# taithenguyen/ppls

Measured on AMD Instinct MI355X. Metric: accepted subintervals/sec + FP64 F-evals/sec at 1/2/4/8 MI355X, EPSILON=1e-10, higher is better.
Workload: dtype f64

## Files before the change

ppls_amd/csrc/aq_shape.h:

```cpp
#pragma once

#if defined(__HIPCC__)
#define AQ_SHAPE_HD __host__ __device__
#else
#define AQ_SHAPE_HD
#endif

namespace aq {

#ifndef AQ_PT
#define AQ_PT 768
#endif
#ifndef AQ_WCAP
#define AQ_WCAP 256
#endif
constexpr int PT = AQ_PT;
constexpr int NW = PT / 64;
constexpr int WCAP = AQ_WCAP;
#ifndef AQ_LONE_NW
#define AQ_LONE_NW 8
#endif
#ifndef AQ_S_W
#define AQ_S_W 2
#endif
constexpr int S_W = AQ_S_W;
#ifndef AQ_S_W1
#define AQ_S_W1 2
#endif
AQ_SHAPE_HD constexpr int seed_depth(unsigned long long V) {
    return V <= 1ull ? AQ_S_W1 : 63 - __builtin_clzll(V) + S_W;
}
AQ_SHAPE_HD constexpr unsigned seed_nb(int D, unsigned long long V) {
    if (V <= 1ull) return 1u << D;
    unsigned nb = 1u << (D - (63 - __builtin_clzll(V)));
    while (nb > 1u && (unsigned long long)(nb - 1u) * V >= (1ull << D)) --nb;
    return nb;
}
AQ_SHAPE_HD constexpr int seed_depth_job(unsigned long long V) {
    return (unsigned long long)(seed_depth(V) + 2) * seed_nb(seed_depth(V) + 1, V) <= 64ull
        ? seed_depth(V) + 1 : seed_depth(V);
}
constexpr int PCU_MAXK = 12;
constexpr int STATIC_MAXK = 16;
constexpr int MAXK = 1 << 18;
constexpr int NSLOTS = MAXK;
constexpr int SYNC_SLOT = NSLOTS;
constexpr int NPARTS = 16384;
#ifndef AQ_GSPLIT_DEFAULT
#define AQ_GSPLIT_DEFAULT 192
#endif
constexpr int DEFAULT_GSPLIT = AQ_GSPLIT_DEFAULT;
// ... 14 lines not shown
```

ppls_amd/csrc/aq_stream.h:

```cpp
#pragma once
#include "aq_device.h"
#include "aq_shape.h"
#include "aq_xsum.h"

namespace aq {

typedef double f64x2 __attribute__((ext_vector_type(2)));

constexpr int PCAP = 128;
constexpr int DT_STRIDE = 2;
constexpr int LREC = NW * WCAP + PCAP;
constexpr int POOL0 = NW * WCAP;
constexpr int CH = PCAP;
struct DtField {
    unsigned* p;
    __device__ __forceinline__ unsigned& operator[](unsigned j) const { return p[DT_STRIDE * j]; }
    __device__ __forceinline__ DtField operator+(unsigned o) const { return DtField{p + DT_STRIDE * o}; }
};
#ifndef AQ_JOB_RUN_MAX
#define AQ_JOB_RUN_MAX 16
#endif
constexpr int JOB_RUN_MAX = AQ_JOB_RUN_MAX;
#ifndef AQ_GSS_DIV
#define AQ_GSS_DIV 2
#endif
constexpr unsigned GSS_DIV = AQ_GSS_DIV;
#ifndef AQ_HEAP_SEED
#define AQ_HEAP_SEED 1
#endif
constexpr bool HEAP_SEED = AQ_HEAP_SEED != 0;
constexpr int HEAP_D = 4;
constexpr unsigned HEAP_NODES = (2u << HEAP_D) - 1u;
static_assert(HEAP_NODES + 2u <= 64u, "the heap seeding path is one node per lane");
__device__ __forceinline__ unsigned div_small(unsigned q, unsigned nb, float rnb) {
    unsigned d = (unsigned)((float)q * rnb);
    d += (d + 1u) * nb <= q ? 1u : 0u;
    d -= d * nb > q ? 1u : 0u;
    return d;
}
#ifndef AQ_GIVE_MIN
#define AQ_GIVE_MIN 96
#endif
constexpr int GIVE_MIN = AQ_GIVE_MIN;
constexpr int DONATE_MIN = 64;
#ifndef AQ_POLL_ROUNDS
// ... 189 lines not shown
    unsigned long long* cu_acc;
    Chunk* chunks;
    Cellar* cellar;
    unsigned* ready;
    LaunchHint* hint;
    int per_cu;
    int static_jobs;
    double2 kbounds[PCU_MAXK];
    int adaptive;
    const double* theta;
};
static_assert(sizeof(StreamParams) == 384, "the kernels' hidden arguments follow the block: a larger one moves them in every instance");

enum : int {
    DG_T_START = 0, DG_T_SEEDED, DG_T_FIRST_LEAD, DG_T_EXIT, DG_ROUNDS, DG_TASKS, DG_CHUNKS_OUT, DG_CHUNKS_IN,
    DG_RECORDS_OUT, DG_T_WAIT, DG_LEADS, DG_SEEDS, DG_POOL_PUSH, DG_CU, DG_RECORDS_IN, DG_ACTIVE_LANES,
    DG_C_ROUND, DG_C_EVAL, DG_POOL_TAKE, DG_LOCK_SPINS, DG_T_LAST_ROUND, DG_SPILL_RECORDS, DG_MAX_RING, DG_C_SEED,
    DG_SEED_CALLS, DG_FLUSHES, DG_MAX_CELLAR, DG_C_IDLE, DG_C_LOCK, DG_C_SHARE, DG_GIVE, DG_CELLAR_IN,
    DG_CELLAR_OUT, DG_C_REFILL, DG_C_LOOP, DG_ACTIVE_TASKS, DG_PREFETCH, DG_T_INIT, DG_T_DONE, DG_T_FOLD,
    DG_T_BROKE, DG_T_FLUSHED, DG_C_P1_CLASS, DG_C_P1_WALK, DG_C_P1_F, DG_T_SEED_IN, DG_T_CLASS, DG_POLLS,
    DIAG_WORDS = 48
};

struct WgState {
    int lock;
    unsigned pbot, ptop;
    int idle;
    int phase;
    int busy_token;
    unsigned exited;
    unsigned long long tasks;
};

struct LdsPairs {
    double* a;
    double* b;
    double* fa;
    double* fm;
    double* fb;
    DtField dt;
};

__device__ __forceinline__ void wave_lock(int* lock, unsigned lane, unsigned long long& spins) {
    if (lane == 0) {
        int expect = 0;
        while (!__hip_atomic_compare_exchange_strong(lock, &expect, 1, __ATOMIC_ACQUIRE, __ATOMIC_RELAXED,
                                                     __HIP_MEMORY_SCOPE_WORKGROUP)) {
            expect = 0;
            ++spins;
            __builtin_amdgcn_s_sleep(1);
        }
    }
    __builtin_amdgcn_wave_barrier();
    __builtin_amdgcn_fence(__ATOMIC_ACQUIRE, "workgroup");
}

__device__ __forceinline__ void wave_unlock(int* lock, unsigned lane) {
    __builtin_amdgcn_fence(__ATOMIC_RELEASE, "workgroup");
    __builtin_amdgcn_wave_barrier();
    if (lane == 0) __hip_atomic_store(lock, 0, __ATOMIC_RELEASE, __HIP_MEMORY_SCOPE_WORKGROUP);
    __builtin_amdgcn_wave_barrier();
}

__device__ __forceinline__ void copy_pair(const LdsPairs& R, unsigned i, unsigned j) {
    const double a = R.a[i], b = R.b[i], fa = R.fa[i], fm = R.fm[i], fb = R.fb[i];
    const unsigned dt = R.dt[i];
    R.a[j] = a; R.b[j] = b; R.fa[j] = fa; R.fm[j] = fm; R.fb[j] = fb; R.dt[j] = dt;
}

template <typename SrcIdx>
__device__ __forceinline__ void publish_chunk(const StreamParams& P, const LdsPairs& R, unsigned slot, unsigned k,
                                              SrcIdx src, unsigned lane) {
    Chunk* __restrict__ c = P.chunks + slot;
    for (unsigned i = lane; i < k; i += 64) {
        const unsigned j = src(i);
        st_wt(&c->a[i], R.a[j]); st_wt(&c->b[i], R.b[j]);
        st_wt(&c->fa[i], R.fa[j]); st_wt(&c->fm[i], R.fm[j]); st_wt(&c->fb[i], R.fb[j]);
        st_wt(&c->dt[i], R.dt[j]);
    }
    if (lane == 0) st_wt(&c->count, k);
    asm volatile("s_waitcnt vmcnt(0)" ::: "memory");
    if (lane == 0) st_wt(&P.ready[(size_t)slot * READY_STRIDE], P.epoch);
}

struct Acc {
    double hi, lo;
    unsigned tasks, leaves, maxd;
    unsigned ut, ul;
    unsigned maxdt;
    double r = 0.0;
};

template <bool ERR>
struct ErrAcc {};
template <>
struct ErrAcc<true> {
    double sg = 0.0, ab = 0.0;
};

template <int FID, bool PCU, bool ERR = false>
__device__ __forceinline__ void flush_acc(const StreamParams& P, Acc& a, int tag, unsigned lane, WgState& S,
                                          unsigned long long* pc, double2* wdd, int wdd_stride, long long* xsa,
                                          long long* xsb, ErrAcc<ERR>& ea, double2* werr) {
    dd_add(a.hi, a.lo, a.r);
    a.r = 0.0;
    if (uni(a.ut) != 0u || __ballot(a.tasks != 0u) != 0ull) {
        double hi = area_scale<FID>() * a.hi, lo = area_scale<FID>() * a.lo;
#if AQ_FLUSHX == 1
        const unsigned t = a.ut + 1u, l = a.ul, m = 1u;
#elif AQ_FLUSHX == 3
        const unsigned mdt = wave_max_full(a.maxdt);
// ... 86 lines not shown
    const unsigned long long a64 = (unsigned long long)(base + p);
    const unsigned long long addr = ((unsigned long long)(unsigned)__builtin_amdgcn_readfirstlane((int)(a64 >> 32)) << 32) |
                                    (unsigned)__builtin_amdgcn_readfirstlane((int)(unsigned)a64);
    u32x4 r;
    asm volatile("s_load_dwordx4 %0, %1, 0x0\n\ts_waitcnt lgkmcnt(0)" : "=s"(r) : "s"(addr) : "memory");
    return make_double2(__hiloint2double((int)r.y, (int)r.x), __hiloint2double((int)r.w, (int)r.z));
}

typedef unsigned u32x2 __attribute__((ext_vector_type(2)));
template <int FID>
__device__ __forceinline__ void sload_theta(Theta<FID>& th, const double* base, int p) {
    if constexpr (FID == F_PARAM) {
        constexpr int NP = param::nparams;
        const unsigned long long a64 = (unsigned long long)(base + (size_t)p * NP);
        const unsigned long long addr = ((unsigned long long)(unsigned)__builtin_amdgcn_readfirstlane((int)(a64 >> 32)) << 32) |
                                        (unsigned)__builtin_amdgcn_readfirstlane((int)(unsigned)a64);
#pragma unroll
        for (int i = 0; i < NP; i += 2) {
            const unsigned long long ai = addr + 8ull * (unsigned)i;
            if (i + 1 < NP) {
                u32x4 r;
                asm volatile("s_load_dwordx4 %0, %1, 0x0\n\ts_waitcnt lgkmcnt(0)" : "=s"(r) : "s"(ai) : "memory");
                th.v[i] = __hiloint2double((int)r.y, (int)r.x);
                th.v[i + 1 < NP ? i + 1 : i] = __hiloint2double((int)r.w, (int)r.z);
            } else {
                u32x2 r;
                asm volatile("s_load_dwordx2 %0, %1, 0x0\n\ts_waitcnt lgkmcnt(0)" : "=s"(r) : "s"(ai) : "memory");
                th.v[i] = __hiloint2double((int)r.y, (int)r.x);
            }
        }
    }
}

static_assert(LREC * 8 == 50 * 512, "the pair moves assume 50 x 512 B per field");
__device__ __forceinline__ void lds_pop6_masked(unsigned long long m, unsigned addr, unsigned addr2, double& a,
                                                double& b, double& fa, double& fm, double& fb, double& dw) {
    unsigned long long saved;
    asm volatile(
        "s_mov_b64 %6, exec\n\t"
        "s_mov_b64 exec, %7\n\t"
        "ds_read_b64 %0, %8\n\t"
        "ds_read_b64 %1, %8 offset:25600\n\t"
        "ds_read_b64 %2, %8 offset:51200\n\t"
        "ds_read_b64 %3, %9\n\t"
        "ds_read_b64 %4, %9 offset:25600\n\t"
        "ds_read_b64 %5, %9 offset:51200\n\t"
        "s_mov_b64 exec, %6\n\t"
        "s_waitcnt lgkmcnt(0)"
        : "+v"(a), "+v"(b), "+v"(fa), "+v"(fm), "+v"(fb), "+v"(dw), "=&s"(saved)
        : "s"(m), "v"(addr), "v"(addr2)
        : "memory");
}
__device__ __forceinline__ void lds_push6_masked(unsigned long long m, unsigned addr, double x0, double x1, double x2,
                                                 double x3, double x4, double x5) {
    unsigned long long saved;
    asm volatile(
        "s_mov_b64 %0, exec\n\t"
        "s_mov_b64 exec, %1\n\t"
        "ds_write2st64_b64 %2, %3, %4 offset1:50\n\t"
        "ds_write2st64_b64 %2, %5, %6 offset0:100 offset1:150\n\t"
        "ds_write2st64_b64 %2, %7, %8 offset0:200 offset1:250\n\t"
        "s_mov_b64 exec, %0"
        : "=&s"(saved)
        : "s"(m), "v"(addr), "v"(x0), "v"(x1), "v"(x2), "v"(x3), "v"(x4), "v"(x5)
        : "memory");
}
struct PairRegs {
    f64x2 ab, ff, fd;
};
__device__ __forceinline__ void lds_issue6(unsigned addr, PairRegs& r) {
    asm volatile(
        "ds_read2st64_b64 %0, %3 offset1:50\n\t"
        "ds_read2st64_b64 %1, %3 offset0:100 offset1:150\n\t"
        "ds_read2st64_b64 %2, %3 offset0:200 offset1:250"
        : "=&v"(r.ab), "=&v"(r.ff), "=&v"(r.fd)
        : "v"(addr)
        : "memory");
}
__device__ __forceinline__ void lds_wait6(PairRegs& r) {
    asm volatile("s_waitcnt lgkmcnt(0)" : "+v"(r.ab), "+v"(r.ff), "+v"(r.fd) : : "memory");
}
__device__ __forceinline__ void lds_store6(unsigned addr, const PairRegs& r) {
    asm volatile(
        "ds_write2st64_b64 %0, %1, %2 offset1:50\n\t"
        "ds_write2st64_b64 %0, %3, %4 offset0:100 offset1:150\n\t"
        "ds_write2st64_b64 %0, %5, %6 offset0:200 offset1:250"
        :
        : "v"(addr), "v"(r.ab.x), "v"(r.ab.y), "v"(r.ff.x), "v"(r.ff.y), "v"(r.fd.x), "v"(r.fd.y)
        : "memory");
}
__device__ __forceinline__ PairRegs chunk_load(const CellarChunk* ch, unsigned lane) {
    return PairRegs{ch->ab[lane], ch->ff[lane], ch->fd[lane]};
}
__device__ __forceinline__ void chunk_store(CellarChunk* ch, unsigned lane, const PairRegs& r) {
    ch->ab[lane] = r.ab;
    ch->ff[lane] = r.ff;
    ch->fd[lane] = r.fd;
}
__device__ __forceinline__ unsigned ring_addr(unsigned ring8, unsigned i, unsigned vmask) {
    return ((i << 3) & vmask) | ring8;
}
__device__ __forceinline__ unsigned ring_slot(unsigned i) { return i % (unsigned)WCAP; }
__device__ __forceinline__ unsigned ring_wrap(unsigned v) {
    if constexpr ((WCAP & (WCAP - 1)) == 0) return v & (unsigned)(WCAP - 1);
    else return min(v, v - (unsigned)WCAP);
}

#if AQ_STAMPS
__device__ unsigned long long g_aq_stamps[MAXG * NW * ST_STRIDE];
#endif

template <int FID, bool HIST, bool DIAG, bool PCU, int NWT = NW, bool HEAPS = false, bool ERR = false>
__global__ __launch_bounds__(NWT * 64) void k_stream(StreamParams P) {
    static_assert(!ERR || (!HIST && !DIAG), "ERR launches keep no histograms and no diagnostics");
    constexpr int PTT = NWT * 64;
    static_assert(NWT >= 4 && NWT <= NW && NWT % 4 == 0, "whole waves per SIMD, within the LDS rings");
    static_assert(NWT <= 16, "the exit's area sum runs over one DPP row of lanes (PCU_AREA)");
    constexpr bool WIDE = AQ_WIDE_TAB && FID == F_COSH4 && !PCU;
    constexpr int TAB_FRONT = WIDE ? 256 * 16 / 8 : 0;
    __shared__ double s_lds[TAB_FRONT + 6 * LREC];
    double* const s_pr = s_lds + TAB_FRONT;
    __shared__ ExpEntry tab_own[WIDE ? 1 : ftab_entries<FID>()];
    ExpEntry* const tab = WIDE ? reinterpret_cast<ExpEntry*>(s_lds) : tab_own;
    const DtField s_dt{reinterpret_cast<unsigned*>(s_pr + 5 * LREC)};
    double* const s_a = s_pr;
    double* const s_b = s_pr + LREC;
    double* const s_fa = s_pr + 2 * LREC;
    double* const s_fm = s_pr + 3 * LREC;
    double* const s_fb = s_pr + 4 * LREC;
    __shared__ WgState S;
    __shared__ unsigned long long s_pc[PCU ? 3 * PCU_ROW : 1];
    __shared__ double2 s_wdd[PCU ? PCU_ROW * NWT : 1];
    __shared__ double2 s_werr[PCU && ERR ? PCU_ROW * NWT : 1];
    __shared__ unsigned long long s_dg[DIAG ? DIAG_WORDS : 1];

    const unsigned tid = threadIdx.x;
    const unsigned lane = lane_id();
    const unsigned wid = __builtin_amdgcn_readfirstlane(tid >> 6);
    const unsigned bid = __builtin_amdgcn_readfirstlane(blockIdx.x);
    QCtl* __restrict__ qc = P.q;
    const LdsPairs R{s_a, s_b, s_fa, s_fm, s_fb, s_dt};
    const unsigned pr_base = (unsigned)(uintptr_t)s_pr;
    const unsigned long long t_entry = (DIAG || AQ_STAMPS) ? rtc() : 0ull;
    unsigned long long stp[ST_N] = {};
    auto stamp = [&](int k) {
        if constexpr (AQ_STAMPS && !DIAG) { if (!stp[k]) stp[k] = rtc(); }
    };
    stp[ST_ENTRY] = t_entry;
    if constexpr (AQ_STAMPS && !DIAG) {
        asm volatile("" :: "s"(P.eps), "s"(P.shares), "s"(P.nprob), "s"(P.kbounds[0].x));
        stamp(ST_KARG);
    }
    ExpPair tv{};
    if (FID != F_SIN_RECIP && tid < (WIDE ? 256u : 128u)) tv = reinterpret_cast<const ExpPair*>(kExpTabBits)[tid & 127u];
    static_assert(FID != F_SIN_RECIP || AQ_SINCOS_TAB_N <= PTT, "one sin-table entry per thread");
    double sv = 0.0;
    if (FID == F_SIN_RECIP && tid < (unsigned)AQ_SINCOS_TAB_N) sv = kSinCosTab[tid];
    stamp(ST_PRE);
    if (bid == 0)
        for (unsigned i = tid; i < (unsigned)(sizeof(QCtl) / 4); i += PTT) reinterpret_cast<unsigned*>(P.q_next)[i] = 0u;
    if (tid == 0) {
        S.lock = 0; S.pbot = 0; S.ptop = 0; S.idle = 0; S.phase = 0; S.busy_token = 1;
        S.exited = 0; S.tasks = 0;
    }
    if (PCU && tid < 3u * PCU_ROW) s_pc[tid] = 0ull;
    if (PCU)
        for (unsigned i = tid; i < (unsigned)(PCU_ROW * NWT); i += PTT) s_wdd[i] = make_double2(0.0, 0.0);
    if constexpr (PCU && ERR)
        for (unsigned i = tid; i < (unsigned)(PCU_ROW * NWT); i += PTT) s_werr[i] = make_double2(0.0, 0.0);
    if (DIAG) {
        for (unsigned i = tid; i < DIAG_WORDS; i += PTT) s_dg[i] = (i == DG_T_FIRST_LEAD) ? ~0ull : 0ull;
    }
    if (FID == F_SIN_RECIP) {
        if (tid < (unsigned)AQ_SINCOS_TAB_N) reinterpret_cast<double*>(tab)[tid] = sv;
// ... 7 lines not shown

    const double eps = P.eps;
    const double eps2 = eps / area_scale<FID>();
    const int max_depth = P.max_depth;
    unsigned shares_main = (unsigned)P.shares;
    int D_main = P.D;
    unsigned long long per_hint = 0;
    if (!PCU && (P.adaptive & 1)) {
        unsigned h = uni(__hip_atomic_load(&P.hint->shares_next, __ATOMIC_RELAXED, __HIP_MEMORY_SCOPE_AGENT));
        if (h) {
            if constexpr (HEAPS) {
                const unsigned long long per =
                    (P.adaptive & 4) ? __hip_atomic_load(&P.hint->per_next, __ATOMIC_RELAXED, __HIP_MEMORY_SCOPE_AGENT)
                                     : (h >= 2u ? (unsigned long long)h * TASKS_PER_JOB : 0ull);
                const unsigned fill = (gridDim.x * (unsigned)NWT + (unsigned)P.nprob - 1u) / (unsigned)P.nprob;
                const unsigned long long cap = per / MIN_JOB_TASKS;
                h = uni(max(h, (unsigned)min((unsigned long long)fill, cap)));
                per_hint = per;
            }
            shares_main = h;
            D_main = seed_depth_job((unsigned long long)h * (unsigned long long)P.nshards);
        }
    }
    const unsigned W = gridDim.x * (unsigned)NWT;
    const unsigned w_all = bid * (unsigned)NWT + wid;
    const unsigned grp = bid % (unsigned)NGROUP;
    const unsigned grp_size = (gridDim.x - grp + (unsigned)NGROUP - 1u) / (unsigned)NGROUP;
    const int t0 = (int)min(gridDim.x, (unsigned)NGROUP);
    const unsigned tail_from = (!PCU && shares_main >= 8u) ? (unsigned)P.tail_from : (unsigned)P.nprob;
    const unsigned shares_tail = min(shares_main * (unsigned)P.tail_mult, W);
    const int D_tail = seed_depth_job((unsigned long long)shares_tail * (unsigned long long)P.nshards);
    const unsigned main_jobs = tail_from * shares_main;
    const unsigned total_jobs = main_jobs + ((unsigned)P.nprob - tail_from) * shares_tail;
    const unsigned base = wid * WCAP;
    long long* const xs_a = reinterpret_cast<long long*>(s_a + base + (WCAP - 64));
    long long* const xs_b = reinterpret_cast<long long*>(s_b + base + (WCAP - 64));
    const unsigned ring8 = pr_base + base * 8u;
    __builtin_assume((ring8 & (unsigned)(WCAP * 8 - 1)) == 0u);
    unsigned ring_vmask = (unsigned)((WCAP - 1) << 3);
    asm volatile("" : "+v"(ring_vmask));

    Acc acc{0.0, 0.0, 0u, 0u, 0u, 0u, 0u, 0u};
    ErrAcc<ERR> eacc;
    auto err_leaf = [&](double d) {
        if constexpr (ERR) {
            eacc.sg += d / area_scale<FID>();
            eacc.ab += fabs(d) / area_scale<FID>();
        }
    };
    int tag = 0;
    Theta<FID> th{};
    sload_theta<FID>(th, P.theta, tag);
    unsigned ctop = 0;
    Cellar* __restrict__ cel = P.cellar + w_all;
    const bool static_jobs = PCU || P.static_jobs != 0;
    unsigned job = (static_jobs || HEAPS) ? wid * gridDim.x + bid : w_all;
    bool job_pending = false;
    unsigned claim = 0;
    unsigned jpc = (!static_jobs && shares_main == 1u && P.nshards == 1 && JOB_RUN_MAX > 1)
                       ? max(1u, min((unsigned)JOB_RUN_MAX, total_jobs / (4u * W)))
                       : 1u;
    if constexpr (HEAPS) {
        if (per_hint) jpc = uni(max(1u, min(jpc, (unsigned)min((unsigned long long)TASKS_PER_JOB / per_hint, 64ull))));
    }
    unsigned job_end = job + 1u;
    unsigned claim_n = jpc;
    unsigned err = 0;
    bool mixed = false;
    unsigned top = 0, bot = 0;
    bool counted_idle = false;
// ... 83 lines not shown
                }
            }
            if (job_pending) {
                job = W + uni(__shfl(claim, 0, 64));
                job_end = job + claim_n;
                job_pending = false;

            }
            unsigned k = 0;
            int ptag = 0;
            bool lead = false, seed = false;
            int phase = 0;
            bool counted_now = false;
            const bool pool_empty = uni(__hip_atomic_load(&S.ptop, __ATOMIC_RELAXED, __HIP_MEMORY_SCOPE_WORKGROUP)) ==
                                    uni(__hip_atomic_load(&S.pbot, __ATOMIC_RELAXED, __HIP_MEMORY_SCOPE_WORKGROUP));
            if (job < total_jobs && (fresh || pool_empty)) {
                seed = true;
            } else if (!counted_idle && !job_pending && job >= total_jobs && pool_empty) {
                stamp(ST_IDLE);
                unsigned old = 0;
                if (lane == 0) old = __hip_atomic_fetch_add(&S.idle, 1, __ATOMIC_RELAXED, __HIP_MEMORY_SCOPE_WORKGROUP);
                old = uni(__shfl(old, 0, 64));
                counted_idle = true;
                counted_now = old + 1u != (unsigned)NWT;
            }
            if (!seed && !counted_now) {
                wave_lock(&S.lock, lane, lock_spins);
                {
                    const unsigned avail = uni(S.ptop - S.pbot);
                    phase = uni(S.phase);
                    if (avail > 0) {
                        k = min(avail, (unsigned)REFILL);
                        const unsigned pb = S.pbot;
                        ptag = (int)uni(dt_tag(s_dt[POOL0 + (pb & (PCAP - 1))]));
                        for (unsigned q0 = 0; q0 < k; q0 += 64) {
                            const unsigned q = q0 + lane;
                            const unsigned long long bad =
                                __ballot(q < k && (int)dt_tag(s_dt[POOL0 + ((pb + q) & (PCAP - 1))]) != ptag);
                            if (bad) {
                                k = q0 + (unsigned)__builtin_ctzll(bad);
                                break;
                            }
                        }
                        for (unsigned i = lane; i < k; i += 64) copy_pair(R, POOL0 + ((pb + i) & (PCAP - 1)), base + i);
                        if (lane == 0) {
                            S.pbot = pb + k;
                            if (counted_idle) __hip_atomic_fetch_add(&S.idle, -1, __ATOMIC_RELAXED, __HIP_MEMORY_SCOPE_WORKGROUP);
                        }
                        __builtin_amdgcn_wave_barrier();
                        counted_idle = false;
                    } else if (job < total_jobs) {
                        seed = true;
                    } else {
                        if (!counted_idle) {
                            stamp(ST_IDLE);
                            if (lane == 0) __hip_atomic_fetch_add(&S.idle, 1, __ATOMIC_RELAXED, __HIP_MEMORY_SCOPE_WORKGROUP);
                            __builtin_amdgcn_wave_barrier();
                            counted_idle = true;
                        }
                        __builtin_amdgcn_wave_barrier();
                        if (phase == 0 && uni(__hip_atomic_load(&S.idle, __ATOMIC_RELAXED, __HIP_MEMORY_SCOPE_WORKGROUP)) == NWT) {
                            lead = true;
                            if (lane == 0) S.phase = 1;
                            __builtin_amdgcn_wave_barrier();
                        }
                    }
                }
                wave_unlock(&S.lock, lane);
            }
            fresh = false;
            if constexpr (DIAG) {
                if (lane == 0) {
                    if (k) atomicAdd(&s_dg[DG_POOL_TAKE], (unsigned long long)k);
                    atomicAdd(&s_dg[DG_C_IDLE], clk() - ci);
                }
            }
            if (k) {
// ... 43 lines not shown
                    for (unsigned d = 0; d < nlev; ++d) col0 |= 1ull << (d * nb);
                    colmask = uni(col0) << (lane - div_small(lane, nb, nb_rcp) * nb);
                }
                unsigned long long cf0 = 0;
                if constexpr (AQ_STAMPS && !DIAG) cf0 = clk();
                if (p != tag) {
                    flush_acc<FID, PCU, ERR>(P, acc, tag, lane, S, s_pc, s_wdd + wid, NWT, xs_a, xs_b, eacc, s_werr + wid);
                    tag = p;
                    sload_theta<FID>(th, P.theta, tag);
                }
                if constexpr (AQ_STAMPS && !DIAG) {
                    const unsigned long long cf1 = clk();
                    stp[ST_CF] += cf1 - cf0;
                    cf0 = cf1;
                }
                const double2 ab = PCU ? P.kbounds[p] : sload_bounds(P.bounds, p);
                if constexpr (AQ_STAMPS && !DIAG) stp[ST_CBD] += clk() - cf0;
                if (static_jobs) {
                    job += W;
                } else if (total_jobs > W) {
                    if (job + 1u < job_end) {
                        ++job;
                    } else {
                        const unsigned left = total_jobs > job + 1u ? total_jobs - job - 1u : 0u;
                        claim_n = jpc > 1u && GSS_DIV ? max(1u, min(jpc, left / (GSS_DIV * W))) : jpc;
                        if (lane == 0) claim = g_add(&qc->jobs.v, claim_n);
                        job_pending = true;
                    }
                } else {
                    job = total_jobs;
                }
                const double A = ab.x, B = ab.y;
                if constexpr (AQ_STAMPS && !DIAG) { asm volatile("" :: "s"(A)); stamp(ST_CLASS); }
                double* fm = s_a + base;
                double* leafa = s_b + base;
                const DtField flag = s_dt + base;
                [[maybe_unused]] double* dleafa = s_fa + base;
                auto position = [&](unsigned kk, bool& valid) -> unsigned long long {
                    const unsigned long long o = (kk & 1u) ? (unsigned long long)(V - 1 - vw) : (unsigned long long)vw;
                    const unsigned long long j = (unsigned long long)kk * V + o;
                    valid = j < npos_total;
                    return j;
                };
                unsigned long long cp1 = 0, cp2 = 0;
                bool alive = false, alive2 = false;
                double l = A, r = B, fl = 0.0, fr = 0.0, mid = 0.0, fmid = 0.0;
                double l2 = A, r2 = B, fl2 = 0.0, fr2 = 0.0, fmid2 = 0.0;
                int Ds = D;
                if (HEAP_SEED && HEAPS && V == 1u) {
                    Ds = HEAP_D;
                    const unsigned q = lane;
                    const bool isnode = q < HEAP_NODES;
                    const unsigned d = isnode ? 31u - (unsigned)__builtin_clz(q + 1u) : 0u;
                    const unsigned k = isnode ? q + 1u - (1u << d) : 0u;
                    unsigned li = HEAP_NODES, ri = HEAP_NODES + 1u;
                    for (unsigned i = 0; i < d; ++i) {
                        const double mm = (l + r) / 2;
                        const unsigned anc = (1u << i) - 1u + (k >> (d - i));
                        if ((k >> (d - 1u - i)) & 1u) { l = mm; li = anc; } else { r = mm; ri = anc; }
                    }
                    mid = (l + r) / 2;
                    if (q < HEAP_NODES + 2u) {
                        fmid = integrand<FID>(isnode ? mid : (q == HEAP_NODES ? A : B), tab, th);
                        fm[q] = fmid;
                    }
                    __builtin_amdgcn_wave_barrier();
                    bool refine = false;
                    double leafarea = 0.0;
                    [[maybe_unused]] double dleaf = 0.0;
                    if (isnode) {
// ... 242 lines not shown
                            if ((pp & ((1ull << (D - (int)d)) - 1ull)) == 0ull) {
                                ++acc.tasks;
                                acc.maxd = max(acc.maxd, d + 1u);
                                if (HIST) atomicAdd(&P.ctls[P.first_slot + p].hist[d], 1ull);
                                if (d == dstar) {
                                    dd_add(acc.hi, acc.lo, leafa[d * nb + kk] / area_scale<FID>());
                                    ++acc.leaves;
                                    if constexpr (ERR) err_leaf(dleafa[d * nb + kk]);
                                    if (HIST) atomicAdd(&P.ctls[P.first_slot + p].hist[AQ_MAX_LEVELS + d], 1ull);
                                } else if ((int)d + 1 >= max_depth) {
                                    err |= ERRB_DEPTH;
                                }
                            }
                        }
                        alive = dstar >= nlev && D + 1 < max_depth;
                        if (burst_cap && alive) acc.maxd = max(acc.maxd, (unsigned)D + 2u);
                        if (alive) {
                            unsigned li = nnodes, ri = nnodes + 1;
                            for (int i = 0; i < D; ++i) {
                                const double mm = (l + r) / 2;
                                if ((pp >> (D - 1 - i)) & 1ull) { l = mm; li = (unsigned)i * nb + kk; } else { r = mm; ri = (unsigned)i * nb + kk; }
                            }
                            fl = fm[li];
                            fr = fm[ri];
                            mid = (l + r) / 2;
                            fmid = fm[(unsigned)D * nb + kk];
                        }
                    }
                }
                __builtin_amdgcn_wave_barrier();
                const unsigned long long am = __ballot(alive);
                constexpr double fs = f_scale<FID>();
                if (alive) {
                    const unsigned j = base + mbcnt(am);
                    s_a[j] = 0.5 * l; s_b[j] = 0.5 * r; s_fa[j] = fs * fl; s_fm[j] = fs * fmid; s_fb[j] = fs * fr;
                    const bool span = FID == F_COSH4 && cosh_main_span(l, r);
                    s_dt[j] = (unsigned)(Ds + 1) | (span ? SPAN_BIT : 0u) | ((unsigned)p << TAG_SHIFT);
                }
                unsigned n_seeds = (unsigned)__popcll(am);
                if constexpr (FID == F_SIN_RECIP) {
                    const unsigned long long am2 = __ballot(alive2);
                    if (alive2) {
                        const unsigned j = base + n_seeds + mbcnt(am2);
                        s_a[j] = 0.5 * l2; s_b[j] = 0.5 * r2; s_fa[j] = fs * fl2; s_fm[j] = fs * fmid2; s_fb[j] = fs * fr2;
                        s_dt[j] = (unsigned)(D + 1) | ((unsigned)p << TAG_SHIFT);
                    }
                    n_seeds += (unsigned)__popcll(am2);
                }
                bot = 0;
                top = n_seeds;
                stamp(ST_SEEDED);
                if constexpr (AQ_STAMPS && !DIAG) {
                    stp[ST_CS] += clk() - cs_st;
                    stp[ST_NS] += 1ull;
                }
                if constexpr (DIAG) {
                    if (lane == 0) {
                        atomicAdd(&s_dg[DG_SEED_CALLS], 1ull);
                        atomicAdd(&s_dg[DG_C_LOCK], cp1 - cs);
                        atomicAdd(&s_dg[DG_C_SHARE], cp2 - cp1);
                        atomicAdd(&s_dg[DG_FLUSHES], clk() - cp2);
                        atomicAdd(&s_dg[DG_SEEDS], (unsigned long long)top);
                        atomicAdd(&s_dg[DG_C_SEED], clk() - cs);
                        atomicMax(&s_dg[DG_T_SEEDED], rtc());
                    }
                }
                __builtin_amdgcn_wave_barrier();
                continue;
            }

            if (phase == 2) break;
            unsigned r_idle = 0;
            bool had_token = false;
            if (lead && lane == 0) {
                had_token = S.busy_token != 0;
                if (had_token) {
                    S.busy_token = 0;
                    r_idle = g_add(&qc->idle[grp].v, 1u);
// ... 47 lines not shown
                            const unsigned tl = g_ld(&qc->tail.v);
                            const unsigned long long now = rtc();
                            if (tk != seen_tk || tl != seen_tl) {
                                seen_tk = tk;
                                seen_tl = tl;
                                t_prog = now;
                            } else if (now - t_prog > P.stall_ticks) {
                                err |= ERRB_TIMEOUT;
                                cmd = -2;
                                break;
                            }
                        }
                        __builtin_amdgcn_s_sleep(AQ_LEAD_SLEEP);
                    }
                }
                if (cmd >= 0) {
                    __builtin_amdgcn_fence(__ATOMIC_ACQUIRE, "wavefront");
                    cnt = ld_wt(&P.chunks[cmd].count);
                }
            }
            cmd = uni(__shfl(cmd, 0, 64));
            cnt = uni(__shfl(cnt, 0, 64));
            if constexpr (DIAG) { if (lane == 0 && cmd < 0) atomicMax(&s_dg[DG_T_DONE], rtc()); }
            if (cmd < 0) stamp(ST_DONE);
            if (cmd < 0) {
                if (lane == 0) __hip_atomic_store(&S.phase, 2, __ATOMIC_RELAXED, __HIP_MEMORY_SCOPE_WORKGROUP);
                __builtin_amdgcn_wave_barrier();
                break;
            }
            const Chunk* __restrict__ c = P.chunks + cmd;
            wave_lock(&S.lock, lane, lock_spins);
            const unsigned pt = uni(S.ptop);
            for (unsigned i = lane; i < cnt; i += 64) {
                const unsigned j = POOL0 + ((pt + i) & (PCAP - 1));
                s_a[j] = ld_wt(&c->a[i]); s_b[j] = ld_wt(&c->b[i]);
                s_fa[j] = ld_wt(&c->fa[i]); s_fm[j] = ld_wt(&c->fm[i]); s_fb[j] = ld_wt(&c->fb[i]);
                s_dt[j] = ld_wt(&c->dt[i]);
            }
            if (lane == 0) {
                S.ptop = pt + cnt;
                S.phase = 0;
                S.busy_token = 1;
                __hip_atomic_fetch_add(&S.idle, -1, __ATOMIC_RELAXED, __HIP_MEMORY_SCOPE_WORKGROUP);
                const bool was_all_idle = g_add(&qc->idle[grp].v, ~0u) == grp_size;
                g_add((int*)&qc->tokens.v, (was_all_idle ? 1 : 0) - (int)(cnt + 1u));
            }
            counted_idle = false;
            wave_unlock(&S.lock, lane);
            if constexpr (DIAG) {
                if (lane == 0) {
                    atomicAdd(&s_dg[DG_CHUNKS_IN], 1ull);
                    atomicAdd(&s_dg[DG_RECORDS_IN], (unsigned long long)cnt);
                    atomicAdd(&s_dg[DG_T_WAIT], rtc() - tl);
                }
            }
            __builtin_amdgcn_wave_barrier();
            continue;
        }

        if (size > (unsigned)(WCAP - 64)) {
            if (pf_n) {
                ctop += pf_n;
                pf_n = 0;
            }
            if (ctop + (unsigned)SPILL <= (unsigned)CCAP) {
                spill_to_cellar(bot, ctop);
                ctop += (unsigned)SPILL;
                bot += (unsigned)SPILL;
                __builtin_amdgcn_wave_barrier();
                continue;
            }
            wave_lock(&S.lock, lane, lock_spins);
            const unsigned pt = uni(S.ptop);
            const bool fits = (pt - S.pbot) + 64u <= (unsigned)PCAP;
            if (fits) {
                copy_pair(R, base + ring_slot(bot + lane), POOL0 + ((pt + lane) & (PCAP - 1)));
                if (lane == 0) S.ptop = pt + 64u;
            }
            wave_unlock(&S.lock, lane);
            if (!fits) {
                unsigned slot = 0;
                if (lane == 0) {
                    slot = g_add(&qc->tail.v, 1u);
                    if (slot < P.qcap) g_add((int*)&qc->tokens.v, 64 + 1);
                    spilled += 64;
                }
                slot = uni(__shfl(slot, 0, 64));
                if (slot < P.qcap) {
                    const unsigned b = bot;
                    publish_chunk(P, R, slot, 64u, [&](unsigned i) { return base + ring_slot(b + i); }, lane);
                } else {
                    err |= ERRB_OVERFLOW;
                }
            }
            if constexpr (DIAG) { if (lane == 0) atomicAdd(&s_dg[DG_POOL_PUSH], 64ull); }
            bot += 64;
            __builtin_amdgcn_wave_barrier();
            continue;
        }

        ++poll_ctr;
        if ((poll_ctr % poll_rounds) == 0) {
            unsigned slot = 0xffffffffu;
            if (lane == 0) {
                if constexpr (DIAG) atomicAdd(&s_dg[DG_POLLS], 1ull);
                if ((int)(seen_head - seen_tail) > 0) {
                    unsigned expect = seen_tail;
                    if (__hip_atomic_compare_exchange_strong(&qc->tail.v, &expect, seen_tail + 1u, __ATOMIC_RELAXED,
                                                             __ATOMIC_RELAXED, __HIP_MEMORY_SCOPE_AGENT))
                        slot = seen_tail;
                    if constexpr (DIAG) atomicAdd(&s_dg[DG_POLLS], 1ull << 32);
                }
                seen_head = g_ld(&qc->head.v);
                seen_tail = g_ld(&qc->tail.v);
            }
            slot = uni(__shfl(slot, 0, 64));
            if (slot != 0xffffffffu) {
                if (slot >= P.qcap) {
                    err |= ERRB_OVERFLOW;
                } else {
                    wave_lock(&S.lock, lane, lock_spins);
                    const unsigned pavail = uni(S.ptop - S.pbot);
                    unsigned k;
                    if (pavail >= (unsigned)DONATE_MIN) {
                        k = min((unsigned)CH, pavail / 2u);
                        const unsigned pb = S.pbot;
                        if (lane == 0) g_add((int*)&qc->tokens.v, (int)k + 1);
                        publish_chunk(P, R, slot, k, [&](unsigned i) { return POOL0 + ((pb + i) & (PCAP - 1)); }, lane);
                        if (lane == 0) S.pbot = pb + k;
                        wave_unlock(&S.lock, lane);
                    } else {
                        wave_unlock(&S.lock, lane);
                        k = size / 2u;
                        if (lane == 0) g_add((int*)&qc->tokens.v, (int)k + 1);
                        const unsigned b = bot;
                        publish_chunk(P, R, slot, k, [&](unsigned i) { return base + ring_slot(b + i); }, lane);
                        bot += k;
                    }
                    if (lane == 0) spilled += k;
                    if constexpr (DIAG) {
                        if (lane == 0) {
                            atomicAdd(&s_dg[DG_CHUNKS_OUT], 1ull);
                            atomicAdd(&s_dg[DG_RECORDS_OUT], (unsigned long long)k);
                        }
                    }
                    __builtin_amdgcn_wave_barrier();
                    continue;
                }
            }
        }

        if ((poll_ctr % give_rounds) == 0 && size >= give_min &&
            uni(__hip_atomic_load(&S.idle, __ATOMIC_RELAXED, __HIP_MEMORY_SCOPE_WORKGROUP)) > 0 &&
            uni(__hip_atomic_load(&S.ptop, __ATOMIC_RELAXED, __HIP_MEMORY_SCOPE_WORKGROUP)) ==
                uni(__hip_atomic_load(&S.pbot, __ATOMIC_RELAXED, __HIP_MEMORY_SCOPE_WORKGROUP))) {
            const unsigned k = size / 2u;
            wave_lock(&S.lock, lane, lock_spins);
            const unsigned pt = uni(S.ptop);
            const bool fits = (pt - S.pbot) + k <= (unsigned)PCAP;
            if (fits) {
                for (unsigned i = lane; i < k; i += 64)
                    copy_pair(R, base + ring_slot(bot + i), POOL0 + ((pt + i) & (PCAP - 1)));
                if (lane == 0) S.ptop = pt + k;
            }
            wave_unlock(&S.lock, lane);
            if constexpr (DIAG) { if (lane == 0) atomicAdd(&s_dg[DG_GIVE], (unsigned long long)(fits ? k : 0u)); }
            if (fits) {
                bot += k;
                __builtin_amdgcn_wave_barrier();
                continue;
            }
        }
        if (ctop > 0 && pf_n == 0 && size <= (unsigned)PF_ISSUE) {
            pf_n = 64u;
            ctop -= pf_n;
            pf = chunk_load(&cel->c[ctop / 64u], lane);
            __builtin_amdgcn_wave_barrier();
        }

        unsigned long long cb0 = 0;
        if constexpr (AQ_STAMPS && !DIAG) cb0 = clk();
        unsigned b_top = uni(top), b_size = uni(size), b_poll = uni(poll_ctr);
        unsigned b_n = 0;
        unsigned long long b_dv = 0;
        unsigned b_bot = uni(bot), b_ctop = uni(ctop), b_pf = uni(pf_n);
        bool b_mixed = uni(mixed);
        unsigned b_S = b_size, b_S0 = b_size;
        unsigned long long b_am = 0;
        double ca = 0.0, cb = 0.0, cfa = 0.0, cfm = 0.0, cfb = 0.0, cdw = 0.0;
        unsigned b_lo1, b_span;
        auto window = [&]() {
            b_lo1 = (b_pf != 0u ? (unsigned)PF_BELOW : (b_ctop > 0u ? (unsigned)PF_ISSUE : 0u)) + 1u;
            b_span = (unsigned)(WCAP - 64) + 1u - b_lo1;
        };
        window();
        constexpr bool prio_by_load = PCU && FID == F_SIN_RECIP;
        const bool b_heavy = prio_by_load && b_S >= HEAVY_S;
        const unsigned b_max = give_rounds - b_poll % give_rounds;
        unsigned b_rem = b_max;
        __builtin_amdgcn_s_waitcnt(0xC07F);
        bool b_go;
        for (;;) {
        for (;;) {
            unsigned long long c0 = 0, c1 = 0;
            if constexpr (DIAG) c0 = clk();
            if constexpr (prio_by_load) {
                if (b_heavy) asm volatile("s_setprio 3");
                else asm volatile("s_setprio 1");
            }
            const unsigned long long need = ~b_am;
            const unsigned k = min((unsigned)__popcll(need), b_top - b_bot);
            const unsigned jr = mbcnt(need);
            const unsigned long long fmsk = __ballot(jr < k) & need;
            b_top -= k;
            const unsigned paddr = ring_addr(ring8, ring_slot(b_top) + jr, ring_vmask);
            lds_pop6_masked(fmsk, paddr, paddr + 3u * 50u * 512u, ca, cb, cfa, cfm, cfb, cdw);
            const unsigned long long am = b_am | fmsk;
            const unsigned na = (unsigned)__popcll(am);
            const double pa = ca, pb = cb, pfa = cfa, pfm = cfm, pfb = cfb;
            const unsigned long long dtw = (unsigned long long)__double_as_longlong(cdw);
            const unsigned dt = (unsigned)dtw;
            using StepT = typename std::conditional<ERR, Step2e, Step2>::type;
            StepT st[2];
            unsigned long long nospan = 0ull;
            if constexpr (FID == F_COSH4) nospan = __ballot((int)dt >= 0);
            double pm, hm;
            pair_step_halves<FID, WIDE ? 255u : 127u, StepT>(pa, pb, pfa, pfm, pfb, eps2, tab, st, pm, hm, kk,
                                                              FID == F_COSH4 ? 2 : -1, nospan & am, th);
            if constexpr (prio_by_load) { if (!b_heavy) asm volatile("s_setprio 0"); }
            const unsigned long long r0m = __ballot(st[0].refine), r1m = __ballot(st[1].refine);
            unsigned long long okm = am;
            if constexpr (!burst_cap) {
                const unsigned long long dm = __ballot((dt & 255u) < (unsigned)(max_depth - 1));
                okm = am & dm;
                const unsigned long long atcap = am & ~dm;
                if (__builtin_expect(atcap != 0ull, 0)) b_dv |= atcap & (r0m | r1m);
            }
            const unsigned long long l0m = am & ~r0m, l1m = am & ~r1m;
            b_n += na;
            const unsigned long long mask0 = okm & r0m, mask1 = okm & r1m;
            const unsigned cdt = dt + 1u;
            const unsigned long long cdtw = ((dtw >> 32) << 32) | (unsigned long long)cdt;
            masked_acc3(acc.r, st[0].area2, l0m, st[1].area2, l1m, acc.maxdt, burst_cap ? cdt : dt,
                        burst_cap ? (mask0 | mask1) : am);
            if constexpr (ERR) masked_err4(eacc.sg, eacc.ab, st[0].diff, l0m, st[1].diff, l1m);
            if constexpr (DIAG) {
                const int rtag = (int)dt_tag(dt);
                b_mixed |= (__ballot(rtag != tag) & am) != 0ull;
            }
// ... 229 lines not shown
```

Baseline: 300.9 billion.

## Lay out LDS pair fields per wave ring instead of globally planar

Reorganizes the shared-memory pair storage so each wave's ring holds its six fields in a contiguous block with a 2 KiB field stride, followed by a shared pool block, instead of six global planes each spanning all rings and the pool. Pop, push and issue now use a single base address with small immediate offsets, which removes the second address register and its add from the hot pop path. It may also change LDS bank-conflict behaviour across waves. Copy and publish helpers become templated on the plane stride.

Result: no change. 301.2 billion (median of 6 runs) (+0.1%).

```diff
diff --git a/ppls_amd/csrc/aq_shape.h b/ppls_amd/csrc/aq_shape.h
--- a/ppls_amd/csrc/aq_shape.h
+++ b/ppls_amd/csrc/aq_shape.h
@@ -17,6 +17,39 @@
 constexpr int PT = AQ_PT;
 constexpr int NW = PT / 64;
 constexpr int WCAP = AQ_WCAP;
+
+constexpr int LDS_FIELDS = 6;
+constexpr int PCAP = 128;
+constexpr unsigned LDS_BYTES = 160u * 1024u;
+constexpr unsigned LDS_WIDE_TAB_BYTES = 256u * 16u;
+constexpr unsigned RING_FIELD_STRIDE = (unsigned)WCAP * 8u;
+constexpr unsigned POOL_FIELD_STRIDE = (unsigned)PCAP * 8u;
+constexpr unsigned RING_BYTES = LDS_FIELDS * RING_FIELD_STRIDE;
+constexpr unsigned POOL_BYTES = LDS_FIELDS * POOL_FIELD_STRIDE;
+AQ_SHAPE_HD constexpr unsigned lds_pairs_base(bool wide) { return wide ? LDS_WIDE_TAB_BYTES : 0u; }
+AQ_SHAPE_HD constexpr unsigned lds_ring_off(unsigned wave, unsigned field, unsigned slot) {
+    return wave * RING_BYTES + field * RING_FIELD_STRIDE + slot * 8u;
+}
+constexpr unsigned LDS_POOL_OFF = (unsigned)NW * RING_BYTES;
+AQ_SHAPE_HD constexpr unsigned lds_pool_off(unsigned field, unsigned slot) {
+    return LDS_POOL_OFF + field * POOL_FIELD_STRIDE + slot * 8u;
+}
+constexpr unsigned LDS_PAIRS_BYTES = LDS_POOL_OFF + POOL_BYTES;
+AQ_SHAPE_HD constexpr unsigned lds_misc_off(bool wide) { return lds_pairs_base(wide) + LDS_PAIRS_BYTES; }
+AQ_SHAPE_HD constexpr unsigned lds_misc_bytes(bool wide) { return LDS_BYTES - lds_misc_off(wide); }
+AQ_SHAPE_HD constexpr unsigned lds_ring_addr(unsigned ring8, unsigned i) {
+    return ((i << 3) & ((unsigned)(WCAP - 1) << 3)) | ring8;
+}
+static_assert((WCAP & (WCAP - 1)) == 0 && (PCAP & (PCAP - 1)) == 0, "ring and pool indices wrap by a mask");
+static_assert((LDS_FIELDS - 1) * RING_FIELD_STRIDE <= 65535u - 8u,
+              "every field of a ring slot within one ds_read_b64 offset of the slot's first");
+static_assert(RING_FIELD_STRIDE % 512u == 0u && (LDS_FIELDS - 1) * RING_FIELD_STRIDE / 512u <= 255u,
+              "every field of a ring slot at a whole ds_*2st64_b64 offset");
+static_assert(RING_BYTES % RING_FIELD_STRIDE == 0u && LDS_WIDE_TAB_BYTES % RING_FIELD_STRIDE == 0u,
+              "a ring's block starts at a multiple of its field stride (lds_ring_addr's and-or)");
+static_assert(lds_misc_off(true) + 1024u <= LDS_BYTES && lds_misc_off(false) + 1024u <= LDS_BYTES,
+              "tables and pairs within a CU's LDS, with room for the workgroup's other words");
+
 #ifndef AQ_LONE_NW
 #define AQ_LONE_NW 8
 #endif
diff --git a/ppls_amd/csrc/aq_stream.h b/ppls_amd/csrc/aq_stream.h
--- a/ppls_amd/csrc/aq_stream.h
+++ b/ppls_amd/csrc/aq_stream.h
@@ -7,10 +7,7 @@
 
 typedef double f64x2 __attribute__((ext_vector_type(2)));
 
-constexpr int PCAP = 128;
 constexpr int DT_STRIDE = 2;
-constexpr int LREC = NW * WCAP + PCAP;
-constexpr int POOL0 = NW * WCAP;
 constexpr int CH = PCAP;
 struct DtField {
     unsigned* p;
@@ -266,14 +263,20 @@
     unsigned long long tasks;
 };
 
-struct LdsPairs {
-    double* a;
-    double* b;
-    double* fa;
-    double* fm;
-    double* fb;
-    DtField dt;
+template <unsigned FS>
+struct LdsPlanes {
+    double* p;
+    __device__ __forceinline__ double& a(unsigned i) const { return p[i]; }
+    __device__ __forceinline__ double& b(unsigned i) const { return p[FS + i]; }
+    __device__ __forceinline__ double& fa(unsigned i) const { return p[2u * FS + i]; }
+    __device__ __forceinline__ double& fm(unsigned i) const { return p[3u * FS + i]; }
+    __device__ __forceinline__ double& fb(unsigned i) const { return p[4u * FS + i]; }
+    __device__ __forceinline__ DtField dtf() const { return DtField{reinterpret_cast<unsigned*>(p + 5u * FS)}; }
+    __device__ __forceinline__ unsigned& dt(unsigned i) const { return dtf()[i]; }
 };
+using RingPlanes = LdsPlanes<(unsigned)WCAP>;
+using PoolPlanes = LdsPlanes<(unsigned)PCAP>;
+static_assert(RING_FIELD_STRIDE == 8u * WCAP && POOL_FIELD_STRIDE == 8u * PCAP, "LdsPlanes restates aq_shape.h's strides");
 
 __device__ __forceinline__ void wave_lock(int* lock, unsigned lane, unsigned long long& spins) {
     if (lane == 0) {
@@ -296,21 +299,22 @@
     __builtin_amdgcn_wave_barrier();
 }
 
-__device__ __forceinline__ void copy_pair(const LdsPairs& R, unsigned i, unsigned j) {
-    const double a = R.a[i], b = R.b[i], fa = R.fa[i], fm = R.fm[i], fb = R.fb[i];
-    const unsigned dt = R.dt[i];
-    R.a[j] = a; R.b[j] = b; R.fa[j] = fa; R.fm[j] = fm; R.fb[j] = fb; R.dt[j] = dt;
-}
-
-template <typename SrcIdx>
-__device__ __forceinline__ void publish_chunk(const StreamParams& P, const LdsPairs& R, unsigned slot, unsigned k,
+template <unsigned FS, unsigned FD>
+__device__ __forceinline__ void copy_pair(const LdsPlanes<FS>& S, unsigned i, const LdsPlanes<FD>& D, unsigned j) {
+    const double a = S.a(i), b = S.b(i), fa = S.fa(i), fm = S.fm(i), fb = S.fb(i);
+    const unsigned dt = S.dt(i);
+    D.a(j) = a; D.b(j) = b; D.fa(j) = fa; D.fm(j) = fm; D.fb(j) = fb; D.dt(j) = dt;
+}
+
+template <unsigned FS, typename SrcIdx>
+__device__ __forceinline__ void publish_chunk(const StreamParams& P, const LdsPlanes<FS>& R, unsigned slot, unsigned k,
                                               SrcIdx src, unsigned lane) {
     Chunk* __restrict__ c = P.chunks + slot;
     for (unsigned i = lane; i < k; i += 64) {
         const unsigned j = src(i);
-        st_wt(&c->a[i], R.a[j]); st_wt(&c->b[i], R.b[j]);
-        st_wt(&c->fa[i], R.fa[j]); st_wt(&c->fm[i], R.fm[j]); st_wt(&c->fb[i], R.fb[j]);
-        st_wt(&c->dt[i], R.dt[j]);
+        st_wt(&c->a[i], R.a(j)); st_wt(&c->b[i], R.b(j));
+        st_wt(&c->fa[i], R.fa(j)); st_wt(&c->fm[i], R.fm(j)); st_wt(&c->fb[i], R.fb(j));
+        st_wt(&c->dt[i], R.dt(j));
     }
     if (lane == 0) st_wt(&c->count, k);
     asm volatile("s_waitcnt vmcnt(0)" ::: "memory");
@@ -463,23 +467,23 @@
     }
 }
 
-static_assert(LREC * 8 == 50 * 512, "the pair moves assume 50 x 512 B per field");
-__device__ __forceinline__ void lds_pop6_masked(unsigned long long m, unsigned addr, unsigned addr2, double& a,
+static_assert(RING_FIELD_STRIDE == 2048u, "the pair moves' offsets are written out for 2 KiB between a ring's fields");
+__device__ __forceinline__ void lds_pop6_masked(unsigned long long m, unsigned addr, double& a,
                                                 double& b, double& fa, double& fm, double& fb, double& dw) {
     unsigned long long saved;
     asm volatile(
         "s_mov_b64 %6, exec\n\t"
         "s_mov_b64 exec, %7\n\t"
         "ds_read_b64 %0, %8\n\t"
-        "ds_read_b64 %1, %8 offset:25600\n\t"
-        "ds_read_b64 %2, %8 offset:51200\n\t"
-        "ds_read_b64 %3, %9\n\t"
-        "ds_read_b64 %4, %9 offset:25600\n\t"
-        "ds_read_b64 %5, %9 offset:51200\n\t"
+        "ds_read_b64 %1, %8 offset:2048\n\t"
+        "ds_read_b64 %2, %8 offset:4096\n\t"
+        "ds_read_b64 %3, %8 offset:6144\n\t"
+        "ds_read_b64 %4, %8 offset:8192\n\t"
+        "ds_read_b64 %5, %8 offset:10240\n\t"
         "s_mov_b64 exec, %6\n\t"
         "s_waitcnt lgkmcnt(0)"
         : "+v"(a), "+v"(b), "+v"(fa), "+v"(fm), "+v"(fb), "+v"(dw), "=&s"(saved)
-        : "s"(m), "v"(addr), "v"(addr2)
+        : "s"(m), "v"(addr)
         : "memory");
 }
 __device__ __forceinline__ void lds_push6_masked(unsigned long long m, unsigned addr, double x0, double x1, double x2,
@@ -488,9 +492,9 @@
     asm volatile(
         "s_mov_b64 %0, exec\n\t"
         "s_mov_b64 exec, %1\n\t"
-        "ds_write2st64_b64 %2, %3, %4 offset1:50\n\t"
-        "ds_write2st64_b64 %2, %5, %6 offset0:100 offset1:150\n\t"
-        "ds_write2st64_b64 %2, %7, %8 offset0:200 offset1:250\n\t"
+        "ds_write2st64_b64 %2, %3, %4 offset1:4\n\t"
+        "ds_write2st64_b64 %2, %5, %6 offset0:8 offset1:12\n\t"
+        "ds_write2st64_b64 %2, %7, %8 offset0:16 offset1:20\n\t"
         "s_mov_b64 exec, %0"
         : "=&s"(saved)
         : "s"(m), "v"(addr), "v"(x0), "v"(x1), "v"(x2), "v"(x3), "v"(x4), "v"(x5)
@@ -501,9 +505,9 @@
 };
 __device__ __forceinline__ void lds_issue6(unsigned addr, PairRegs& r) {
     asm volatile(
-        "ds_read2st64_b64 %0, %3 offset1:50\n\t"
-        "ds_read2st64_b64 %1, %3 offset0:100 offset1:150\n\t"
-        "ds_read2st64_b64 %2, %3 offset0:200 offset1:250"
+        "ds_read2st64_b64 %0, %3 offset1:4\n\t"
+        "ds_read2st64_b64 %1, %3 offset0:8 offset1:12\n\t"
+        "ds_read2st64_b64 %2, %3 offset0:16 offset1:20"
         : "=&v"(r.ab), "=&v"(r.ff), "=&v"(r.fd)
         : "v"(addr)
         : "memory");
@@ -513,9 +517,9 @@
 }
 __device__ __forceinline__ void lds_store6(unsigned addr, const PairRegs& r) {
     asm volatile(
-        "ds_write2st64_b64 %0, %1, %2 offset1:50\n\t"
-        "ds_write2st64_b64 %0, %3, %4 offset0:100 offset1:150\n\t"
-        "ds_write2st64_b64 %0, %5, %6 offset0:200 offset1:250"
+        "ds_write2st64_b64 %0, %1, %2 offset1:4\n\t"
+        "ds_write2st64_b64 %0, %3, %4 offset0:8 offset1:12\n\t"
+        "ds_write2st64_b64 %0, %5, %6 offset0:16 offset1:20"
         :
         : "v"(addr), "v"(r.ab.x), "v"(r.ab.y), "v"(r.ff.x), "v"(r.ff.y), "v"(r.fd.x), "v"(r.fd.y)
         : "memory");
@@ -548,29 +552,25 @@
     static_assert(NWT >= 4 && NWT <= NW && NWT % 4 == 0, "whole waves per SIMD, within the LDS rings");
     static_assert(NWT <= 16, "the exit's area sum runs over one DPP row of lanes (PCU_AREA)");
     constexpr bool WIDE = AQ_WIDE_TAB && FID == F_COSH4 && !PCU;
-    constexpr int TAB_FRONT = WIDE ? 256 * 16 / 8 : 0;
-    __shared__ double s_lds[TAB_FRONT + 6 * LREC];
+    constexpr int TAB_FRONT = (int)(lds_pairs_base(WIDE) / 8u);
+    __shared__ double s_lds[TAB_FRONT + LDS_PAIRS_BYTES / 8u];
     double* const s_pr = s_lds + TAB_FRONT;
     __shared__ ExpEntry tab_own[WIDE ? 1 : ftab_entries<FID>()];
     ExpEntry* const tab = WIDE ? reinterpret_cast<ExpEntry*>(s_lds) : tab_own;
-    const DtField s_dt{reinterpret_cast<unsigned*>(s_pr + 5 * LREC)};
-    double* const s_a = s_pr;
-    double* const s_b = s_pr + LREC;
-    double* const s_fa = s_pr + 2 * LREC;
-    double* const s_fm = s_pr + 3 * LREC;
-    double* const s_fb = s_pr + 4 * LREC;
     __shared__ WgState S;
     __shared__ unsigned long long s_pc[PCU ? 3 * PCU_ROW : 1];
     __shared__ double2 s_wdd[PCU ? PCU_ROW * NWT : 1];
     __shared__ double2 s_werr[PCU && ERR ? PCU_ROW * NWT : 1];
     __shared__ unsigned long long s_dg[DIAG ? DIAG_WORDS : 1];
+    static_assert(sizeof(tab_own) + sizeof(S) + sizeof(s_pc) + sizeof(s_wdd) + sizeof(s_werr) + sizeof(s_dg) + 5 * 16 <=
+                      lds_misc_bytes(WIDE),
+                  "the workgroup's other words fit behind the pair block");
 
     const unsigned tid = threadIdx.x;
     const unsigned lane = lane_id();
     const unsigned wid = __builtin_amdgcn_readfirstlane(tid >> 6);
     const unsigned bid = __builtin_amdgcn_readfirstlane(blockIdx.x);
     QCtl* __restrict__ qc = P.q;
-    const LdsPairs R{s_a, s_b, s_fa, s_fm, s_fb, s_dt};
     const unsigned pr_base = (unsigned)(uintptr_t)s_pr;
     const unsigned long long t_entry = (DIAG || AQ_STAMPS) ? rtc() : 0ull;
     unsigned long long stp[ST_N] = {};
@@ -644,10 +644,11 @@
     const int D_tail = seed_depth_job((unsigned long long)shares_tail * (unsigned long long)P.nshards);
     const unsigned main_jobs = tail_from * shares_main;
     const unsigned total_jobs = main_jobs + ((unsigned)P.nprob - tail_from) * shares_tail;
-    const unsigned base = wid * WCAP;
-    long long* const xs_a = reinterpret_cast<long long*>(s_a + base + (WCAP - 64));
-    long long* const xs_b = reinterpret_cast<long long*>(s_b + base + (WCAP - 64));
-    const unsigned ring8 = pr_base + base * 8u;
+    const RingPlanes ring{s_pr + lds_ring_off(wid, 0u, 0u) / 8u};
+    const PoolPlanes pool{s_pr + lds_pool_off(0u, 0u) / 8u};
+    long long* const xs_a = reinterpret_cast<long long*>(&ring.a(WCAP - 64));
+    long long* const xs_b = reinterpret_cast<long long*>(&ring.b(WCAP - 64));
+    const unsigned ring8 = pr_base + lds_ring_off(wid, 0u, 0u);
     __builtin_assume((ring8 & (unsigned)(WCAP * 8 - 1)) == 0u);
     unsigned ring_vmask = (unsigned)((WCAP - 1) << 3);
     asm volatile("" : "+v"(ring_vmask));
@@ -797,17 +798,17 @@
                     if (avail > 0) {
                         k = min(avail, (unsigned)REFILL);
                         const unsigned pb = S.pbot;
-                        ptag = (int)uni(dt_tag(s_dt[POOL0 + (pb & (PCAP - 1))]));
+                        ptag = (int)uni(dt_tag(pool.dt(pb & (PCAP - 1))));
                         for (unsigned q0 = 0; q0 < k; q0 += 64) {
                             const unsigned q = q0 + lane;
                             const unsigned long long bad =
-                                __ballot(q < k && (int)dt_tag(s_dt[POOL0 + ((pb + q) & (PCAP - 1))]) != ptag);
+                                __ballot(q < k && (int)dt_tag(pool.dt((pb + q) & (PCAP - 1))) != ptag);
                             if (bad) {
                                 k = q0 + (unsigned)__builtin_ctzll(bad);
                                 break;
                             }
                         }
-                        for (unsigned i = lane; i < k; i += 64) copy_pair(R, POOL0 + ((pb + i) & (PCAP - 1)), base + i);
+                        for (unsigned i = lane; i < k; i += 64) copy_pair(pool, (pb + i) & (PCAP - 1), ring, i);
                         if (lane == 0) {
                             S.pbot = pb + k;
                             if (counted_idle) __hip_atomic_fetch_add(&S.idle, -1, __ATOMIC_RELAXED, __HIP_MEMORY_SCOPE_WORKGROUP);
@@ -917,10 +918,10 @@
                 }
                 const double A = ab.x, B = ab.y;
                 if constexpr (AQ_STAMPS && !DIAG) { asm volatile("" :: "s"(A)); stamp(ST_CLASS); }
-                double* fm = s_a + base;
-                double* leafa = s_b + base;
-                const DtField flag = s_dt + base;
-                [[maybe_unused]] double* dleafa = s_fa + base;
+                double* fm = &ring.a(0);
+                double* leafa = &ring.b(0);
+                const DtField flag = ring.dtf();
+                [[maybe_unused]] double* dleafa = &ring.fa(0);
                 auto position = [&](unsigned kk, bool& valid) -> unsigned long long {
                     const unsigned long long o = (kk & 1u) ? (unsigned long long)(V - 1 - vw) : (unsigned long long)vw;
                     const unsigned long long j = (unsigned long long)kk * V + o;
@@ -1229,18 +1230,18 @@
                 const unsigned long long am = __ballot(alive);
                 constexpr double fs = f_scale<FID>();
                 if (alive) {
-                    const unsigned j = base + mbcnt(am);
-                    s_a[j] = 0.5 * l; s_b[j] = 0.5 * r; s_fa[j] = fs * fl; s_fm[j] = fs * fmid; s_fb[j] = fs * fr;
+                    const unsigned j = mbcnt(am);
+                    ring.a(j) = 0.5 * l; ring.b(j) = 0.5 * r; ring.fa(j) = fs * fl; ring.fm(j) = fs * fmid; ring.fb(j) = fs * fr;
                     const bool span = FID == F_COSH4 && cosh_main_span(l, r);
-                    s_dt[j] = (unsigned)(Ds + 1) | (span ? SPAN_BIT : 0u) | ((unsigned)p << TAG_SHIFT);
+                    ring.dt(j) = (unsigned)(Ds + 1) | (span ? SPAN_BIT : 0u) | ((unsigned)p << TAG_SHIFT);
                 }
                 unsigned n_seeds = (unsigned)__popcll(am);
                 if constexpr (FID == F_SIN_RECIP) {
                     const unsigned long long am2 = __ballot(alive2);
                     if (alive2) {
-                        const unsigned j = base + n_seeds + mbcnt(am2);
-                        s_a[j] = 0.5 * l2; s_b[j] = 0.5 * r2; s_fa[j] = fs * fl2; s_fm[j] = fs * fmid2; s_fb[j] = fs * fr2;
-                        s_dt[j] = (unsigned)(D + 1) | ((unsigned)p << TAG_SHIFT);
+                        const unsigned j = n_seeds + mbcnt(am2);
+                        ring.a(j) = 0.5 * l2; ring.b(j) = 0.5 * r2; ring.fa(j) = fs * fl2; ring.fm(j) = fs * fmid2; ring.fb(j) = fs * fr2;
+                        ring.dt(j) = (unsigned)(D + 1) | ((unsigned)p << TAG_SHIFT);
                     }
                     n_seeds += (unsigned)__popcll(am2);
                 }
@@ -1354,10 +1355,10 @@
             wave_lock(&S.lock, lane, lock_spins);
             const unsigned pt = uni(S.ptop);
             for (unsigned i = lane; i < cnt; i += 64) {
-                const unsigned j = POOL0 + ((pt + i) & (PCAP - 1));
-                s_a[j] = ld_wt(&c->a[i]); s_b[j] = ld_wt(&c->b[i]);
-                s_fa[j] = ld_wt(&c->fa[i]); s_fm[j] = ld_wt(&c->fm[i]); s_fb[j] = ld_wt(&c->fb[i]);
-                s_dt[j] = ld_wt(&c->dt[i]);
+                const unsigned j = (pt + i) & (PCAP - 1);
+                pool.a(j) = ld_wt(&c->a[i]); pool.b(j) = ld_wt(&c->b[i]);
+                pool.fa(j) = ld_wt(&c->fa[i]); pool.fm(j) = ld_wt(&c->fm[i]); pool.fb(j) = ld_wt(&c->fb[i]);
+                pool.dt(j) = ld_wt(&c->dt[i]);
             }
             if (lane == 0) {
                 S.ptop = pt + cnt;
@@ -1396,7 +1397,7 @@
             const unsigned pt = uni(S.ptop);
             const bool fits = (pt - S.pbot) + 64u <= (unsigned)PCAP;
             if (fits) {
-                copy_pair(R, base + ring_slot(bot + lane), POOL0 + ((pt + lane) & (PCAP - 1)));
+                copy_pair(ring, ring_slot(bot + lane), pool, (pt + lane) & (PCAP - 1));
                 if (lane == 0) S.ptop = pt + 64u;
             }
             wave_unlock(&S.lock, lane);
@@ -1410,7 +1411,7 @@
                 slot = uni(__shfl(slot, 0, 64));
                 if (slot < P.qcap) {
                     const unsigned b = bot;
-                    publish_chunk(P, R, slot, 64u, [&](unsigned i) { return base + ring_slot(b + i); }, lane);
+                    publish_chunk(P, ring, slot, 64u, [&](unsigned i) { return ring_slot(b + i); }, lane);
                 } else {
                     err |= ERRB_OVERFLOW;
                 }
@@ -1448,7 +1449,7 @@
                         k = min((unsigned)CH, pavail / 2u);
                         const unsigned pb = S.pbot;
                         if (lane == 0) g_add((int*)&qc->tokens.v, (int)k + 1);
-                        publish_chunk(P, R, slot, k, [&](unsigned i) { return POOL0 + ((pb + i) & (PCAP - 1)); }, lane);
+                        publish_chunk(P, pool, slot, k, [&](unsigned i) { return (pb + i) & (PCAP - 1); }, lane);
                         if (lane == 0) S.pbot = pb + k;
                         wave_unlock(&S.lock, lane);
                     } else {
@@ -1456,7 +1457,7 @@
                         k = size / 2u;
                         if (lane == 0) g_add((int*)&qc->tokens.v, (int)k + 1);
                         const unsigned b = bot;
-                        publish_chunk(P, R, slot, k, [&](unsigned i) { return base + ring_slot(b + i); }, lane);
+                        publish_chunk(P, ring, slot, k, [&](unsigned i) { return ring_slot(b + i); }, lane);
                         bot += k;
                     }
                     if (lane == 0) spilled += k;
@@ -1482,7 +1483,7 @@
             const bool fits = (pt - S.pbot) + k <= (unsigned)PCAP;
             if (fits) {
                 for (unsigned i = lane; i < k; i += 64)
-                    copy_pair(R, base + ring_slot(bot + i), POOL0 + ((pt + i) & (PCAP - 1)));
+                    copy_pair(ring, ring_slot(bot + i), pool, (pt + i) & (PCAP - 1));
                 if (lane == 0) S.ptop = pt + k;
             }
             wave_unlock(&S.lock, lane);
@@ -1536,7 +1537,7 @@
             const unsigned long long fmsk = __ballot(jr < k) & need;
             b_top -= k;
             const unsigned paddr = ring_addr(ring8, ring_slot(b_top) + jr, ring_vmask);
-            lds_pop6_masked(fmsk, paddr, paddr + 3u * 50u * 512u, ca, cb, cfa, cfm, cfb, cdw);
+            lds_pop6_masked(fmsk, paddr, ca, cb, cfa, cfm, cfb, cdw);
             const unsigned long long am = b_am | fmsk;
             const unsigned na = (unsigned)__popcll(am);
             const double pa = ca, pb = cb, pfa = cfa, pfm = cfm, pfb = cfb;
```
